# arpg/Kangaroo

Measured on AMD Instinct MI355X. Metric: kinectfusion_frames_per_sec_640x480_to_512cubed_tsdf, higher is better.
Workload: dtype f32

## Files before the change

include/kfx_debug.h:

```cpp
#ifndef KFX_DEBUG_H
#define KFX_DEBUG_H

#include "kfx.h"

#ifdef __cplusplus
extern "C" {
#endif

int kfx_debug_rmw(const kfx_volume* vol, int variant, kfx_stream stream);

int kfx_debug_div_uniform_check(float b, unsigned long long* d_out, kfx_stream stream);

int kfx_debug_div_core_check(unsigned seed, int per_divisor, unsigned long long* d_out, kfx_stream stream);
int kfx_debug_sqrt_core_check(unsigned long long* d_out, kfx_stream stream);
int kfx_debug_wave_xor_check(unsigned seed, unsigned long long* d_out, kfx_stream stream);

int kfx_debug_summary_export(kfx_sdf_summary* s, float tol, float vref, int fine_shift, void* R_out, void* C_out, int dims_out[12],
                             kfx_stream stream);

int kfx_debug_summary_conditional_builds(kfx_sdf_summary* s, int out[2], kfx_stream stream);

#ifdef __cplusplus
}
#endif
#endif
```

kangaroo_amd/csrc/debug.hip:

```cpp
#include "kfx_device.h"
#include "sampling.h"
#include "../../include/kfx_debug.h"

namespace kfx {

__global__ __launch_bounds__(256) void k_rmw_linear(float4* __restrict__ base, size_t n4)
{
    const size_t stride = (size_t)gridDim.x * blockDim.x;
    for (size_t i = (size_t)blockIdx.x * blockDim.x + threadIdx.x; i < n4; i += stride) {
        float4 c = base[i];
        c.y += 1.0f;
        c.w += 1.0f;
        base[i] = c;
    }
}

template <int ZC>
__global__ __launch_bounds__(256) void k_rmw_brick(unsigned char* vptr, size_t pitch, size_t img_pitch, int X, int Y, int Z)
{
    const int tid = threadIdx.x, lane = tid & 63, wv = tid >> 6;
    const int x0 = (blockIdx.x * 32 + (lane & 31)) * 2;
    const int y = blockIdx.y * 8 + wv * 2 + (lane >> 5);
    const int zbeg = blockIdx.z * ZC, zend = min(zbeg + ZC, Z);
    if (x0 >= X || y >= Y) return;
// ... 242 lines not shown
        if (hipMemcpyAsync(C_out, s->C, (size_t)cv.words * sizeof(unsigned), hipMemcpyDeviceToDevice, st) != hipSuccess || hipStreamSynchronize(st) != hipSuccess)
            return set_error(KFX_E_RANGE, "kfx_debug_summary_export: copy");
        dims_out[11] = (s->h_skippable && s->builds) ? ((volatile int*)s->h_skippable)[(s->builds - 1) % KFX_SUMMARY_RING] : -2;
    }
    return 0;
}

extern "C" int kfx_debug_summary_conditional_builds(kfx_sdf_summary* s, int out[2], kfx_stream stream)
{
    if (!s || !out) return set_error(KFX_E_NULL, "kfx_debug_summary_conditional_builds: null argument");
    hipStream_t st = (hipStream_t)stream;
    if (hipMemcpyAsync(out, s->d_count + 3, 2 * sizeof(int), hipMemcpyDeviceToHost, st) != hipSuccess || hipStreamSynchronize(st) != hipSuccess)
        return set_error(KFX_E_RANGE, "kfx_debug_summary_conditional_builds: copy");
    return 0;
}
```

kangaroo_amd/csrc/kfx_device.h:

```cpp
#pragma once

#include <hip/hip_runtime.h>
#include <stddef.h>
#include <stdint.h>

#include "../../include/kfx.h"
#include "../../include/kfx_extras.h"
#include "../../include/kfx_summary_h.h"

namespace kfx {

struct V3 { float x, y, z; };

__device__ __forceinline__ V3 v3(float x, float y, float z) { return V3{x, y, z}; }
__device__ __forceinline__ V3 operator+(V3 a, V3 b) { return V3{a.x + b.x, a.y + b.y, a.z + b.z}; }
__device__ __forceinline__ V3 operator-(V3 a, V3 b) { return V3{a.x - b.x, a.y - b.y, a.z - b.z}; }
__device__ __forceinline__ V3 operator*(V3 a, float s) { return V3{a.x * s, a.y * s, a.z * s}; }
__device__ __forceinline__ V3 div_cw(V3 a, V3 b) { return V3{a.x / b.x, a.y / b.y, a.z / b.z}; }
__device__ __forceinline__ V3 div_s(V3 a, float s) { const float inv = 1.0f / s; return a * inv; }
__device__ __forceinline__ float dot(V3 a, V3 b) { return a.x * b.x + a.y * b.y + a.z * b.z; }
__device__ __forceinline__ float length(V3 a) { return sqrtf(dot(a, a)); }
__device__ __forceinline__ float lerp(float a, float b, float t) { return a + t * (b - a); }
__device__ __forceinline__ V3 lerp(V3 a, V3 b, float t) { return a + (b - a) * t; }
__device__ __forceinline__ float clampf(float f, float a, float b) { return fmaxf(a, fminf(f, b)); }
// ... 141 lines not shown
    int ny;
    int rw;
    int first;
};
struct ClassView {
    const unsigned* C;
    ClassLevel fine, coarse;
    int words;
    float vref;
    float tol;
    int amb_ok;
    int ox, oy, oz;
    float eps;
    int nx5, nz5, top_n, lds_words;
    int global, top_first;
};
__device__ __forceinline__ unsigned brick_class_mask(const float lo, const float hi, const int state, const float lo_ok, const float hi_ok)
{
    const bool in_band = lo >= lo_ok && hi <= hi_ok;
    return (state == 1 ? 1u : 0u) | ((state == 0 && in_band) ? 2u : 0u) | ((state == 1 || in_band) ? 4u : 0u);
}
inline __host__ __device__ void class_level_up(const int nx, const int ny, const int nz, const int shift, const int first, ClassLevel& L, int& ux, int& uz, int& words)
{
    ux = (nx + 1) >> 1; uz = (nz + 1) >> 1;
    L.shift = shift; L.ny = (ny + 1) >> 1; L.rw = 2 * ((ux + 31) >> 5); L.first = first;
    words = (L.rw * L.ny * uz + 3) & ~3;
}
__device__ __forceinline__ void classes_level_up(unsigned* tab, const ClassLevel& src, int snx, int snz, const ClassLevel& dst, int dnx, int dnz)
{
    const int lane = threadIdx.x & 63;
// ... 23 lines not shown
        const unsigned long long p0 = __ballot(cls & 1), p1 = __ballot(cls & 2);
        if (e < total && (bx & 63) == 0 && (chunks > 1 || bx == 0)) {
            const int sh = chunks > 1 ? 0 : lane;
            const unsigned long long m = (chunks > 1 || lg == 6) ? ~0ull : ((1ull << (1 << lg)) - 1ull);
            const unsigned long long r0 = (p0 >> sh) & m, r1 = (p1 >> sh) & m;
            unsigned* out = tab + dst.first + (bz * dst.ny + by) * dst.rw + (bx >> 6) * 4;
            out[0] = (unsigned)r0; out[1] = (unsigned)r1;
            if ((bx >> 6) * 4 + 2 < dst.rw) { out[2] = (unsigned)(r0 >> 32); out[3] = (unsigned)(r1 >> 32); }
        }
    }
}
int summary_classes_prepare(kfx_sdf_summary* s, float tol, float vref, int fine_shift, hipStream_t stream, int global = 0);
void summary_class_layout(const kfx_sdf_summary* s, int fine_shift, ClassView& cv);
void summary_top_layout(const ClassView& cv, ClassLevel& l6, ClassLevel& l7, int& w6, int& w7);
int summary_view_offset(const kfx_sdf_summary* s, const kfx_volume* view, int* ox, int* oy, int* oz);
}

namespace kfx {
int set_error(int code, const char* what);
int check_launch(const char* what);
int math_mode();
size_t texel_image_bytes(size_t w, size_t h);
int depth_to_vbo_normals_texels(const kfx_image* vbo, const kfx_image* nrm, const kfx_image* depth, const float K[4], float scale,
                                const kfx_image* texels, kfx_stream stream);
int sdf_fuse_slab_texels(const kfx_volume* vol, const kfx_slab* slab, const kfx_image* depth, const kfx_image* norm, const kfx_image* texels,
                         const float T_cw[12], const float K[4], float trunc_dist, float max_w, float mincostheta, unsigned flags, kfx_stream stream);
int sdf_fuse_texels(const kfx_volume* vol, kfx_sdf_summary* summary, const kfx_image* depth, const kfx_image* norm, const kfx_image* texels,
                    const float T_cw[12], const float K[4], float trunc_dist, float max_w, float mincostheta, unsigned flags, kfx_stream stream);
}
```

kangaroo_amd/csrc/raycast.hip:

```cpp
#include <cmath>

#include <hip/hip_fp16.h>

#include "kfx_device.h"
#include "sampling.h"

namespace kfx {

struct RayParams {
    VolView vol;
    V3 size;
    V3 dims1;
    V3 hi2;
    V3 voxel;
    V3 inv_size;
    int fastdiv, off32;
    Pose T;
    Intr K;
    unsigned char *dptr, *nptr, *iptr;
    size_t dpitch, npitch, ipitch;
    int w, h;
    float near, far, trunc;
    int subpix;
    int tile_log2w;
    int wg_log2x;
    int sparse_lanes;
};

__device__ __forceinline__ float phong(const V3 p_c, const V3 n_c)
{
    const float ambient = (float)0.4, diffuse = (float)0.4, specular = (float)0.2;
    const V3 eyedir = div_s(p_c * -1.0f, length(p_c));
    const V3 l0 = v3((float)0.4, (float)0.4, -1.0f);
    const V3 lightdir = div_s(l0, length(l0));
    const float ldotn = dot(lightdir, n_c);
    const V3 lightreflect = n_c * (2 * ldotn) + lightdir * -1.0f;
    const float edotr = fmaxf(0.0f, dot(eyedir, lightreflect));
    const float spec = edotr * edotr * edotr * edotr * edotr * edotr * edotr * edotr * edotr * edotr;
    return ambient + diffuse * ldotn + specular * spec;
}

__device__ __forceinline__ void ray_pixel_of(const RayParams& p, int bx, int by, int tid, int& u, int& v)
{
// ... 21 lines not shown
{
    RayBox b;
    b.c_w = v3(p.T.m[3], p.T.m[7], p.T.m[11]);
    b.ray_c = v3(((float)u - p.K.u0) / p.K.fu, ((float)v - p.K.v0) / p.K.fv, 1.0f);
    b.ray_w = so3_mul(p.T, b.ray_c);
    const V3 ta = div_cw(p.vol.bmin - b.c_w, b.ray_w);
    const V3 tb = div_cw(p.vol.bmax - b.c_w, b.ray_w);
    const V3 tmin = v3(fminf(ta.x, tb.x), fminf(ta.y, tb.y), fminf(ta.z, tb.z));
    const V3 tmax = v3(fmaxf(ta.x, tb.x), fmaxf(ta.y, tb.y), fmaxf(ta.z, tb.z));
    b.max_tmin = fmaxf(fmaxf(fmaxf(tmin.x, tmin.y), tmin.z), p.near);
    b.min_tmax = fminf(fminf(fminf(tmax.x, tmax.y), tmax.z), p.far);
    return b;
}
__device__ __forceinline__ bool enters(const RayBox& b) { return b.max_tmin < b.min_tmax; }

template <typename CELL>
__device__ __forceinline__ V3 normal_c(const RayParams& p, const V3 pos_w)
{
    const V3 g = gradient<CELL>(p, pos_w);
    const float len = length(g);
    const V3 n_w = len > 0 ? div_s(g, len) : v3(0.f, 0.f, 1.f);
    return so3_mul_inv(p.T, n_w);
}

struct RayOut { float* depth; float* shade; float4* normal; };
__device__ __forceinline__ RayOut ray_out(const RayParams& p, const int u, const int v)
{
    return RayOut{reinterpret_cast<float*>(p.dptr + (size_t)v * p.dpitch) + u, reinterpret_cast<float*>(p.iptr + (size_t)v * p.ipitch) + u,
                  reinterpret_cast<float4*>(p.nptr + (size_t)v * p.npitch) + u};
}
__device__ __forceinline__ void write_no_hit(const RayOut& o)
{
    *o.depth = __builtin_nanf("");
    *o.shade = 0.f;
    *o.normal = make_float4(0.f, 0.f, 0.f, 0.f);
}
template <typename CELL, bool COLOR>
__device__ __forceinline__ void write_ray(const RayParams& q, const ColorGeom& cv, const int u, const int v, const float depth)
{
    const RayOut o = ray_out(q, u, v);
    if (depth > 0) {
        const RayBox r = ray_box(q, u, v);
        const V3 n_c = normal_c<CELL>(q, r.c_w + r.ray_w * depth);
        *o.depth = depth;
        if constexpr (COLOR) *o.shade = trilinear<RayC32>(cv, r.c_w + r.ray_w * depth);
        else *o.shade = phong(r.ray_c * depth, n_c);
        *o.normal = make_float4(n_c.x, n_c.y, n_c.z, 1.0f);
    } else {
        write_no_hit(o);
    }
}

__device__ __forceinline__ unsigned touch(unsigned* bitmap, const VolView& v, int x, int y, int z)
{
    const size_t i = ((size_t)z * v.h + y) * v.w + x;
    const unsigned bit = 1u << (i & 31);
    unsigned* word = bitmap + (i >> 5);
    if (*reinterpret_cast<volatile unsigned*>(word) & bit) return 0u;
    return (atomicOr(word, bit) & bit) ? 0u : 1u;
}
__device__ __forceinline__ void touch_sample(unsigned* bitmap, const VolView& vol, const CellPos c, unsigned* cnt)
// ... 50 lines not shown
                if (last_sdf > 0) {
                    if (p.subpix) lambda = lambda + delta * sdf / (last_sdf - sdf);
                    depth = lambda;
                }
                break;
            }
            delta = march_step(sdf, min_delta, p.trunc);
            lambda += delta;
            last_sdf = sdf;
        }
    }

    if constexpr (COUNT) {
        if (depth > 0) touch_gradient(bitmap, p, c_w + ray_w * depth, cnt);
    } else {
        write_ray<CELL, COLOR>(p, cv, u, v, depth);
    }
    return depth > 0 ? depth : __builtin_nanf("");
}

struct TopLevels { ClassLevel lv[2]; int n; };

__device__ __forceinline__ int class_lookup(const unsigned* tab, const ClassLevel& L, int gx, int gy, int gz)
{
    const int bx = gx >> L.shift, by = gy >> L.shift, bz = gz >> L.shift;
    const uint2 w = *reinterpret_cast<const uint2*>(tab + L.first + (bz * L.ny + by) * L.rw + ((bx >> 5) << 1));
    return (int)((w.x >> (bx & 31)) & 1u) | (int)(((w.y >> (bx & 31)) & 1u) << 1);
}

template <typename CELL, bool COLOR, bool COUNT = false, bool GT = false>
__device__ __forceinline__ float raycast_pixel_classes(const RayParams& p, const RayParams& q, const ColorGeom& cv, const int u, const int v, const ClassView& cl_arg, const unsigned* tab,
                                                       const TopLevels& top, unsigned* bitmap = nullptr, unsigned* cnt = nullptr)
{
    constexpr bool PARK = !GT && !COUNT;
    ClassView parked;
    if constexpr (PARK) parked = cl_arg;
    ClassView& clp = parked;
    if constexpr (PARK) {
        clp.fine.shift = in_vgpr(clp.fine.shift); clp.fine.ny = in_vgpr(clp.fine.ny); clp.fine.rw = in_vgpr(clp.fine.rw); clp.fine.first = in_vgpr(clp.fine.first);
        clp.coarse.ny = in_vgpr(clp.coarse.ny); clp.coarse.rw = in_vgpr(clp.coarse.rw); clp.coarse.first = in_vgpr(clp.coarse.first);
        clp.ox = in_vgpr(clp.ox); clp.oy = in_vgpr(clp.oy); clp.oz = in_vgpr(clp.oz);
        clp.eps = in_vgpr(clp.eps); clp.vref = in_vgpr(clp.vref);
    }
    const ClassView& cl = PARK ? parked : cl_arg;
    if (u >= p.w || v >= p.h) return 0.f;

    const RayBox box = ray_box(p, u, v);
    const V3 c_w = box.c_w, ray_w = box.ray_w;
    const float max_tmin = box.max_tmin, min_tmax = box.min_tmax;

    float depth = 0.0f;
    if (max_tmin < min_tmax) {
        float lambda = max_tmin;
        float last_sdf = __builtin_nanf("");
        const float min_delta = p.voxel.x;
        float delta = 0.f;
        const V3 sc = v3(p.dims1.x / p.size.x, p.dims1.y / p.size.y, p.dims1.z / p.size.z);
        const V3 pfA = v3((c_w.x - p.vol.bmin.x) * sc.x, (c_w.y - p.vol.bmin.y) * sc.y, (c_w.z - p.vol.bmin.z) * sc.z);
        const V3 pfB = v3(ray_w.x * sc.x, ray_w.y * sc.y, ray_w.z * sc.z);
        const V3 inv = v3(1.0f / pfB.x, 1.0f / pfB.y, 1.0f / pfB.z);
        const float eps = cl.eps;
        const float step_free = fmaxf(cl.vref, min_delta);
        const float inv_step_free = 1.0f / step_free, inv_trunc = 1.0f / p.trunc;
        const float band = cl.tol * cl.vref;
        bool pending = false;
        float lambda_prev = 0.f;
        bool consult = true;
        float lam_retry = lambda;
        int wait = 0, backoff = 1;
        while (lambda < min_tmax) {
            const bool look = consult && wait == 0 && lambda >= lam_retry;
            CellPos c{};
            typename CELL::InFlight fl;
            if (!look) {
                c = cell_of(p, c_w + ray_w * lambda);
                trilinear_issue<CELL>(fl, p, c);
                if constexpr (COUNT) touch_sample(bitmap, p.vol, c, cnt);
            }
            if (look) {
                if constexpr (COUNT) cnt[1] += 1;
                const float ex = __builtin_fmaf(pfB.x, lambda, pfA.x), ey = __builtin_fmaf(pfB.y, lambda, pfA.y), ez = __builtin_fmaf(pfB.z, lambda, pfA.z);
                const float flx = floorf(ex), fly = floorf(ey), flz = floorf(ez);
                const float lo_f = fminf(fminf(ex - flx, ey - fly), ez - flz), hi_f = fmaxf(fmaxf(ex - flx, ey - fly), ez - flz);
                bool run = false;
                if (fminf(fminf(ex, ey), ez) > eps && ex < p.dims1.x - eps && ey < p.dims1.y - eps && ez < p.dims1.z - eps && lo_f > eps && hi_f < 1.0f - eps) {
                    const int gx = (int)flx + cl.ox, gy = (int)fly + cl.oy, gz = (int)flz + cl.oz;
// ... 8 lines not shown
                            int c6 = class_lookup(tab, top.lv[0], gx, gy, gz);
                            if (c6 == 3 && !cl.amb_ok) c6 = 0;
                            if (c6 != 0) { cls = c6; shift = 6; }
                        }
                        if (cls == 0) {
                            int c5 = class_lookup(cl.C, cl.coarse, gx, gy, gz);
                            if (c5 == 3 && !cl.amb_ok) c5 = 0;
                            if (c5 != 0) { cls = c5; shift = 5; }
                        }
                        if (cls == 0) {
                            cls = class_lookup(cl.C, cl.fine, gx, gy, gz);
                            if (cls == 3 && !cl.amb_ok) cls = 0;
                            shift = cl.fine.shift;
                        }
                    } else {
                    cls = class_lookup(tab, cl.fine, gx, gy, gz);
                    if (cls == 3 && !cl.amb_ok) cls = 0;
                    if (cls != 0 && cl.fine.shift < 5) {
                        int c5 = class_lookup(tab, cl.coarse, gx, gy, gz);
                        if (c5 == 3 && !cl.amb_ok) c5 = 0;
                        if (c5 != 0) { cls = c5; shift = 5; }
                    }
                    if (shift == 5 && cl.top_n > 0) {
                        int c6 = class_lookup(tab, top.lv[0], gx, gy, gz);
                        if (c6 == 3 && !cl.amb_ok) c6 = 0;
                        if (c6 != 0) {
                            cls = c6; shift = 6;
                            if (cl.top_n > 1) {
                                int c7 = class_lookup(tab, top.lv[1], gx, gy, gz);
                                if (c7 == 3 && !cl.amb_ok) c7 = 0;
                                if (c7 != 0) { cls = c7; shift = 7; }
                            }
                        }
                    }
                    }
                    const float L = (float)(1 << shift);
                    const float lox = (float)(((gx >> shift) << shift) - cl.ox), loy = (float)(((gy >> shift) << shift) - cl.oy),
                                loz = (float)(((gz >> shift) << shift) - cl.oz);
                    const float bx = pfB.x >= 0.f ? lox + L - eps : lox + eps, by = pfB.y >= 0.f ? loy + L - eps : loy + eps,
                                bz = pfB.z >= 0.f ? loz + L - eps : loz + eps;
                    const float lam_exit = fminf(fminf((bx - pfA.x) * inv.x, (by - pfA.y) * inv.y), (bz - pfA.z) * inv.z);
                    if (cls != 0) {
                        delta = cls == 1 ? step_free : p.trunc;
                        pending = cls == 3 || (CELL::BYTES == 4 && cls == 1 && cl.tol > 0.f);
                        last_sdf = cls == 1 ? cl.vref : __builtin_nanf("");
// ... 28 lines not shown
                        if constexpr (COUNT) touch_sample(bitmap, p.vol, cell_of(p, c_w + ray_w * lambda_prev), cnt);
                    }
                    if (last_sdf > 0) {
                        if (p.subpix) lambda = lambda + delta * sdf / (last_sdf - sdf);
                        depth = lambda;
                    }
                    break;
                }
                delta = march_step(sdf, min_delta, p.trunc);
                lambda += delta;
                last_sdf = sdf;
                pending = false;
                consult = !(fabsf(sdf - cl.vref) > band);
            }
        }
    }

    if constexpr (COUNT) {
        if (depth > 0) touch_gradient(bitmap, p, c_w + ray_w * depth, cnt);
    } else {
        write_ray<CELL, COLOR>(q, cv, u, v, depth);
    }
    return depth > 0 ? depth : __builtin_nanf("");
}

template <bool GT = false>
__device__ __forceinline__ void classes_stage(const ClassView& cl, unsigned* tab, TopLevels& top)
{
    const uint4* src = reinterpret_cast<const uint4*>(cl.C + (GT ? cl.top_first : 0));
    uint4* dst = reinterpret_cast<uint4*>(tab);
    for (int i = threadIdx.x; i < (cl.lds_words >> 2); i += blockDim.x) dst[i] = src[i];
    ClassLevel l6, l7;
    int nx6, nz6, nx7, nz7, w6, w7;
    const int at = GT ? 0 : cl.words;
    class_level_up(cl.nx5, cl.coarse.ny, cl.nz5, 6, at, l6, nx6, nz6, w6);
    class_level_up(nx6, l6.ny, nz6, 7, at + w6, l7, nx7, nz7, w7);
    if (threadIdx.x == 0) { top.lv[0] = l6; top.lv[1] = l7; top.n = cl.top_n; }
    __syncthreads();
}

__device__ __forceinline__ bool workgroup_any(const bool yes, int* s_any)
{
    const bool wave_any = __ballot(yes) != 0ull;
    if ((threadIdx.x & 63) == 0) s_any[threadIdx.x >> 6] = wave_any ? 1 : 0;
    __syncthreads();
    return (s_any[0] | s_any[1] | s_any[2] | s_any[3]) != 0;
}

template <typename CELL, bool GT = false>
__global__ __launch_bounds__(256) void k_raycast_sdf_classes(const RayParams p, const ClassView cl)
{
    extern __shared__ unsigned s_tab[];
    __shared__ RayParams s_p;
    __shared__ TopLevels s_top;
    __shared__ int s_any[4];
    if (threadIdx.x == 0) s_p = p;
    int u, v;
    const bool carries = ray_lane_pixel(p, p.sparse_lanes, blockIdx.x, blockIdx.y, u, v);
    const bool pixel = carries && u < p.w && v < p.h;
    if constexpr (!GT) {
        if (!workgroup_any(pixel && enters(ray_box(p, u, v)), s_any)) {
            if (pixel) write_no_hit(ray_out(p, u, v));
            return;
        }
    }
    classes_stage<GT>(cl, s_tab, s_top);
    if (!carries) return;
    raycast_pixel_classes<CELL, false, false, GT>(p, s_p, ColorGeom{}, u, v, cl, s_tab, s_top);
}

template <typename CELL, bool COLOR>
__global__ __launch_bounds__(256) void k_raycast_sdf(const RayParams p, const ColorGeom cv)
{
    int u, v;
    if (!ray_lane_pixel(p, p.sparse_lanes, blockIdx.x, blockIdx.y, u, v)) return;
    raycast_pixel<CELL, COLOR>(p, cv, u, v);
}

template <typename CELL>
__global__ __launch_bounds__(256) void k_raycast_sdf_count(const RayParams p, unsigned* __restrict__ bitmap, unsigned long long* __restrict__ counters)
{
    int u, v;
    ray_pixel_of(p, blockIdx.x, blockIdx.y, threadIdx.x, u, v);
    unsigned cnt[4] = {0u, 0u, 0u, 0u}, entered = 0;
    if (u < p.w && v < p.h) {
        entered = enters(ray_box(p, u, v)) ? 1u : 0u;
        raycast_pixel<CELL, false, true>(p, ColorGeom{}, u, v, bitmap, cnt);
    }
    publish_counts(cnt, entered, counters);
}

template <typename CELL, bool GT = false>
__global__ __launch_bounds__(256) void k_raycast_sdf_classes_count(const RayParams p, const ClassView cl, unsigned* __restrict__ bitmap,
                                                                   unsigned long long* __restrict__ counters)
{
    extern __shared__ unsigned s_tab[];
    __shared__ RayParams s_p;
    __shared__ TopLevels s_top;
    if (threadIdx.x == 0) s_p = p;
    classes_stage<GT>(cl, s_tab, s_top);
    int u, v;
    ray_pixel_of(p, blockIdx.x, blockIdx.y, threadIdx.x, u, v);
    unsigned cnt[4] = {0u, 0u, 0u, 0u}, entered = 0;
    if (u < p.w && v < p.h) {
        entered = enters(ray_box(p, u, v)) ? 1u : 0u;
        raycast_pixel_classes<CELL, false, true, GT>(p, s_p, ColorGeom{}, u, v, cl, s_tab, s_top, bitmap, cnt);
    }
    publish_counts(cnt, entered, counters);
    if (blockIdx.x == 0 && blockIdx.y == 0 && threadIdx.x == 0) atomicAdd(&counters[5], (unsigned long long)cl.lds_words * 4ull);
}

constexpr int RAY_MAX_LEVELS = 8;
struct RayLevel {
    unsigned char *dptr, *nptr, *iptr;
    size_t dpitch, npitch, ipitch;
    int w, h;
    Intr K;
    unsigned char* vptr;
    size_t vpitch;
    int first_block, blocks_x;
    int sparse;
};
struct RayLevels {
    RayLevel lv[RAY_MAX_LEVELS];
    int n;
};

__device__ __forceinline__ const RayLevel& level_of(const RayLevels& L, const int block)
{
    int l = 0;
    for (int k = 1; k < L.n; ++k)
        if (block >= L.lv[k].first_block) l = k;
    return L.lv[l];
}
__device__ __forceinline__ RayParams level_params(const RayParams& base, const RayLevel& lv)
{
    RayParams p = base;
    p.dptr = lv.dptr; p.nptr = lv.nptr; p.iptr = lv.iptr;
    p.dpitch = lv.dpitch; p.npitch = lv.npitch; p.ipitch = lv.ipitch;
    p.w = lv.w; p.h = lv.h;
    p.K = lv.K;
    return p;
}
__device__ __forceinline__ void write_vertex(const RayLevel& lv, const RayParams& p, const int u, const int v, const float kz)
{
    if (lv.vptr && u < p.w && v < p.h)
        reinterpret_cast<float4*>(lv.vptr + (size_t)v * lv.vpitch)[u] =
            make_float4(kz * ((float)u - p.K.u0) / p.K.fu, kz * ((float)v - p.K.v0) / p.K.fv, kz, 1.0f);
}

template <typename CELL>
__global__ __launch_bounds__(256) void k_raycast_sdf_levels(const RayParams base, const RayLevels L)
{
    const RayLevel& lv = level_of(L, (int)blockIdx.x);
    const RayParams p = level_params(base, lv);
    const int b = (int)blockIdx.x - lv.first_block;
    int u, v;
    if (!ray_lane_pixel(p, lv.sparse, b % lv.blocks_x, b / lv.blocks_x, u, v)) return;
    write_vertex(lv, p, u, v, raycast_pixel<CELL, false>(p, ColorGeom{}, u, v));
}

template <typename CELL>
__global__ __launch_bounds__(256) void k_raycast_sdf_levels_classes(const RayParams base, const RayLevels L, const ClassView cl)
{
    extern __shared__ unsigned s_tab[];
    __shared__ RayParams s_p;
    __shared__ TopLevels s_top;
    __shared__ int s_any[4];
    const RayLevel& lv = level_of(L, (int)blockIdx.x);
    const RayParams p = level_params(base, lv);
    if (threadIdx.x == 0) s_p = p;
    const int b = (int)blockIdx.x - lv.first_block;
    int u, v;
    const bool carries = ray_lane_pixel(p, lv.sparse, b % lv.blocks_x, b / lv.blocks_x, u, v);
    const bool pixel = carries && u < p.w && v < p.h;
    float kz = __builtin_nanf("");
    if (!workgroup_any(pixel && enters(ray_box(p, u, v)), s_any)) {
        if (!pixel) return;
        write_no_hit(ray_out(p, u, v));
    } else {
        classes_stage(cl, s_tab, s_top);
        if (!carries) return;
        kz = raycast_pixel_classes<CELL, false>(p, s_p, ColorGeom{}, u, v, cl, s_tab, s_top);
    }
    write_vertex(lv, p, u, v, kz);
}

struct SlabRay {
    float* state;
    float* touched;
    float* result;
    int packed;
    int normals_here;
    size_t P;
    int R;
    int v0, v1;
    int* fin;
    int claim_misses;
// ... 151 lines not shown
    p.dpitch = depth->pitch;
    p.npitch = norm->pitch;
    p.ipitch = img->pitch;
    p.w = (int)img->w;
    p.h = (int)img->h;
    p.near = near;
    p.far = far;
    p.trunc = trunc_dist;
    p.subpix = subpix ? 1 : 0;
    p.tile_log2w = 5;
    p.wg_log2x = 1;
    p.sparse_lanes = 0;
    return 0;
}

template <typename CELL>
static int class_view(ClassView& cl, size_t* lds_bytes, int* usable, kfx_sdf_summary* summary, const kfx_volume* vol, const RayParams& p, kfx_stream stream,
                      bool allow_global = true)
{
    *usable = 0;
    if (int e = summary_view_offset(summary, vol, &cl.ox, &cl.oy, &cl.oz)) return e;
    if (!(p.trunc > 0.f) || !(p.trunc < __builtin_inff())) return 0;
    static const int kb_env = env_int("KFX_RAYCAST_CLASS_KB", 16, 1, 60);
    static const int gt_env = env_int("KFX_RAYCAST_GLOBAL_TABLES", 0);
    static const int top_env = env_int("KFX_RAYCAST_TOP_LEVELS", 2, 0, 2);
    int fine = 3;
    for (; fine < 5; ++fine) {
        summary_class_layout(summary, fine, cl);
        if ((size_t)cl.words * 4 <= (size_t)kb_env * 1024) break;
    }
// ... 32 lines not shown
    const bool steer = force_env == 0 && summary->h_skippable;
    if (steer && summary->plain_calls && (summary->plain_calls++ % 8u) != 0u) return 0;
    if (int e = summary_classes_prepare(summary, tol, vref, fine, (hipStream_t)stream, cl.global)) return e;
    if (steer && summary->builds >= 3) {
        const unsigned ref = (summary->builds - 3) % KFX_SUMMARY_RING;
        (void)hipEventSynchronize(summary->build_done[ref]);
        const int known = ((volatile int*)summary->h_skippable)[ref];
        if (known >= 0 && (long long)known * 4 < summary->n_coarse) {
            if (!summary->plain_calls) summary->plain_calls = 1;
            return 0;
        }
        summary->plain_calls = 0;
    }
    cl.C = summary->C;
    cl.vref = vref;
    cl.amb_ok = fmaxf(vref, p.voxel.x) == p.trunc ? 1 : 0;
    cl.tol = tol;
    const double u24 = 1.0 / 16777216.0;
    double eps = 0.0;
    const float bmin[3] = {p.vol.bmin.x, p.vol.bmin.y, p.vol.bmin.z}, bmax[3] = {p.vol.bmax.x, p.vol.bmax.y, p.vol.bmax.z};
    const float size[3] = {p.size.x, p.size.y, p.size.z}, dims1[3] = {p.dims1.x, p.dims1.y, p.dims1.z};
    const float cw[3] = {p.T.m[3], p.T.m[7], p.T.m[11]};
    for (int a = 0; a < 3; ++a) {
        if (!(size[a] > 0.f)) return 0;
        const double sc = (double)dims1[a] / size[a];
        const double pmax = std::fmax(std::fabs((double)bmin[a]), std::fabs((double)bmax[a])), ca = std::fabs((double)cw[a]);
        const double A = std::fabs(((double)cw[a] - bmin[a]) * sc);
        const double t = sc * (3.0 * pmax + 2.0 * ca + size[a]) * u24 + 2.0 * dims1[a] * u24;
        const double e = u24 * (3.0 * A + 2.0 * sc * (pmax + ca) + dims1[a]) + 3.0 * u24 * (dims1[a] + A);
        eps = std::fmax(eps, t + e);
// ... 3 lines not shown
    cl.eps = (float)std::fmax(eps, 1e-4);
    *lds_bytes = (size_t)cl.lds_words * sizeof(unsigned);
    *usable = 1;
    return 0;
}

template <typename PLAIN, typename... A>
static int launch_march(const char* what, int usable, const ClassView& cl, size_t cl_bytes, dim3 grid, kfx_stream stream, const RayParams& p,
                        void (*global)(RayParams, ClassView, A...), void (*lds)(RayParams, ClassView, A...), PLAIN plain, A... a)
{
    if (usable) hipLaunchKernelGGL(cl.global ? global : lds, grid, dim3(256), cl_bytes, (hipStream_t)stream, p, cl, a...);
    else plain();
    return check_launch(what);
}

template <typename CELL>
static int raycast_levels_launch(int n_levels, const kfx_image* const* depth, const kfx_image* const* norm, const kfx_image* const* img,
                                 const kfx_image* const* vbo, const kfx_volume* vol, const float T_wc[12], const float* K, float near, float far,
                                 float trunc_dist, int subpix, kfx_stream stream, kfx_sdf_summary* summary = nullptr)
{
    if (n_levels < 0 || n_levels > RAY_MAX_LEVELS) return set_error(KFX_E_RANGE, "RaycastSdf(levels): number of levels");
    if (!depth || !norm || !img || !K) return set_error(KFX_E_NULL, "RaycastSdf(levels): null argument");
    RayParams base{};
    RayLevels L{};
    int blocks = 0;
    for (int l = 0; l < n_levels; ++l) {
        RayParams p;
        if (int e = ray_params<CELL>(p, depth[l], norm[l], img[l], vol, T_wc, K + 4 * l, near, far, trunc_dist, subpix)) return e;
        if (p.w == 0 || p.h == 0) continue;
        RayLevel& lv = L.lv[L.n++];
// ... 298 lines not shown
}

extern "C" int kfx_raycast_state_to_images(const kfx_image* depth, const kfx_image* norm, const kfx_image* img, const float* state,
                                           kfx_stream stream)
{
    if (!depth || !norm || !img || !state || !depth->ptr || !norm->ptr || !img->ptr) return set_error(KFX_E_NULL, "raycast state: null argument");
    if (img->w == 0 || img->h == 0) return 0;
    if (depth->w < img->w || depth->h < img->h || norm->w < img->w || norm->h < img->h) return set_error(KFX_E_SHAPE, "raycast state: image sizes");
    RayParams p{};
    p.dptr = (unsigned char*)depth->ptr; p.nptr = (unsigned char*)norm->ptr; p.iptr = (unsigned char*)img->ptr;
    p.dpitch = depth->pitch; p.npitch = norm->pitch; p.ipitch = img->pitch;
    p.w = (int)img->w; p.h = (int)img->h;
    hipLaunchKernelGGL(k_raycast_state_to_images, dim3(ceil_div(p.w, 64), ceil_div(p.h, 4)), dim3(256), 0, (hipStream_t)stream, p, state);
    return check_launch("kfx_raycast_state_to_images");
}
```

kangaroo_amd/csrc/sampling.h:

```cpp
#pragma once

#include <hip/hip_fp16.h>

#include "kfx_device.h"
#include "host_args.h"

namespace kfx {

struct __attribute__((aligned(8))) Pair { float v0, w0, v1, w1; };
struct RayF32 {
    static constexpr int BYTES = 8;
    __device__ static __forceinline__ float2 pair(const unsigned char* row, int x)
    {
        const Pair c = *reinterpret_cast<const Pair*>(row + (size_t)x * 8);
        return make_float2(c.v0, c.v1);
    }
    __device__ static __forceinline__ float val(const unsigned char* row, int x) { return *reinterpret_cast<const float*>(row + (size_t)x * 8); }
    __device__ static __forceinline__ void pair4(const unsigned char* base, size_t o0, size_t o1, size_t o2, size_t o3,
                                                 float2& c0, float2& c1, float2& c2, float2& c3)
    {
        typedef float f4 __attribute__((ext_vector_type(4)));
        f4 a, b, c, d;
        asm volatile("global_load_dwordx4 %0, %4, off\n\t"
                     "global_load_dwordx4 %1, %5, off\n\t"
// ... 195 lines not shown
__device__ __forceinline__ float trilinear_finish(typename CELL::InFlight& f, const CellPos& c)
{
    float2 c00, c10, c01, c11;
    CELL::finish(f, c00, c10, c01, c11);
    return lerp(lerp(lerp(c00.x, c00.y, c.fx), lerp(c10.x, c10.y, c.fx), c.fy),
                lerp(lerp(c01.x, c01.y, c.fx), lerp(c11.x, c11.y, c.fx), c.fy), c.fz);
}

template <typename CELL, typename GEOM>
__device__ __forceinline__ float trilinear(const GEOM& p, const V3 pos_w)
{
    return trilinear_at<CELL>(p, cell_of(p, pos_w));
}

template <typename CELL, typename GEOM>
__device__ __forceinline__ V3 gradient(const GEOM& p, const V3 pos_w)
{
    const V3 pos_v = div_cw(pos_w - p.vol.bmin, p.size);
    const V3 pf = v3(pos_v.x * p.dims1.x, pos_v.y * p.dims1.y, pos_v.z * p.dims1.z);
    const int ix = (int)fmaxf(fminf(p.hi2.x, floorf(pf.x)), 1.f);
    const int iy = (int)fmaxf(fminf(p.hi2.y, floorf(pf.y)), 1.f);
    const int iz = (int)fmaxf(fminf(p.hi2.z, floorf(pf.z)), 1.f);
    const float fx = pf.x - (float)ix, fy = pf.y - (float)iy, fz = pf.z - (float)iz;
    const VolView& v = p.vol;
    float c[2][2][2], mx[2][2], my[2][2], mz[2][2];
#pragma unroll
    for (int dz = 0; dz < 2; ++dz)
#pragma unroll
        for (int dy = 0; dy < 2; ++dy) {
            const unsigned char* r = rowp(v, iy + dy, iz + dz);
            mx[dz][dy] = CELL::val(r, ix - 1);
            const float2 cc = CELL::pair(r, ix);
            c[dz][dy][0] = cc.x;
// ... 14 lines not shown
    V3 g[2][2][2];
#pragma unroll
    for (int dz = 0; dz < 2; ++dz)
#pragma unroll
        for (int dy = 0; dy < 2; ++dy)
#pragma unroll
            for (int dx = 0; dx < 2; ++dx) {
                const float v0 = c[dz][dy][dx];
                const float bx = dx ? c[dz][dy][0] : mx[dz][dy];
                const float by = dy ? c[dz][0][dx] : my[dz][dx];
                const float bz = dz ? c[0][dy][dx] : mz[dy][dx];
                g[dz][dy][dx] = v3(v0 - bx, v0 - by, v0 - bz);
            }
    const V3 deriv = lerp(lerp(lerp(g[0][0][0], g[0][0][1], fx), lerp(g[0][1][0], g[0][1][1], fx), fy),
                          lerp(lerp(g[1][0][0], g[1][0][1], fx), lerp(g[1][1][0], g[1][1][1], fx), fy), fz);
    return div_cw(deriv, p.voxel);
}

template <typename GEOM>
inline void set_shortcuts(GEOM& g)
{
    g.inv_size = V3{1.0f / g.size.x, 1.0f / g.size.y, 1.0f / g.size.z};
    g.fastdiv = div_uniform_safe_host(g.size.x) && div_uniform_safe_host(g.size.y) && div_uniform_safe_host(g.size.z);
    const double span = (double)(g.vol.d - 1) * (double)g.vol.img_pitch + (double)(g.vol.h - 1) * (double)g.vol.pitch + (double)g.vol.w * 16.0;
    static const int enabled = env_int("KFX_SAMPLER_SHORTCUTS", 1);
    g.off32 = enabled && span < 4294967296.0;
    g.fastdiv = enabled && g.fastdiv;
}

template <typename GEOM>
inline void set_geometry(GEOM& g, const kfx_volume* v)
// ... 22 lines not shown
```

Baseline: 2476.

## Prefetch class table early, hoist march quotients, spread params copy across threads

In the class-table raycast kernels, the first chunk of the class table is loaded into registers before the ray-box test and workgroup vote, so global latency overlaps that work before the LDS store. RayParams is now copied to LDS one word per thread instead of by thread 0 alone. Per-ray constants (scale, free step, reciprocals) are computed on the host and passed in ClassView, the ray box is computed once and passed down, and class words for all pyramid levels are loaded together before they are tested. A clock-instrumented debug variant is added behind a compile flag; the prefetch uses more registers and loads table words even for blocks that then exit early.

```diff
diff --git a/include/kfx_debug.h b/include/kfx_debug.h
--- a/include/kfx_debug.h
+++ b/include/kfx_debug.h
@@ -20,6 +20,12 @@
 
 int kfx_debug_summary_conditional_builds(kfx_sdf_summary* s, int out[2], kfx_stream stream);
 
+int kfx_debug_march_clocks(const kfx_image* depth, const kfx_image* norm, const kfx_image* img, const kfx_volume* vol, kfx_sdf_summary* summary,
+                           const float T_wc[12], const float K[4], float near, float far, float trunc_dist, int subpix,
+                           unsigned long long* d_clocks, size_t clock_words, int* waves, kfx_stream stream);
+
+int kfx_debug_march_quotients(const float boxmin[3], const float boxmax[3], const unsigned dims[3], float trunc_dist, float vref, float out[6]);
+
 #ifdef __cplusplus
 }
 #endif
diff --git a/kangaroo_amd/csrc/debug.hip b/kangaroo_amd/csrc/debug.hip
--- a/kangaroo_amd/csrc/debug.hip
+++ b/kangaroo_amd/csrc/debug.hip
@@ -280,3 +280,11 @@
         return set_error(KFX_E_RANGE, "kfx_debug_summary_conditional_builds: copy");
     return 0;
 }
+
+extern "C" int kfx_debug_march_quotients(const float boxmin[3], const float boxmax[3], const unsigned dims[3], float trunc_dist, float vref, float out[6])
+{
+    if (!boxmin || !boxmax || !dims || !out) return set_error(KFX_E_NULL, "kfx_debug_march_quotients: null argument");
+    if (dims[0] < 3 || dims[1] < 3 || dims[2] < 3) return set_error(KFX_E_SHAPE, "kfx_debug_march_quotients: a volume has at least 3 cells per axis");
+    march_quotients_of(boxmin, boxmax, dims, trunc_dist, vref, out);
+    return 0;
+}
diff --git a/kangaroo_amd/csrc/kfx_device.h b/kangaroo_amd/csrc/kfx_device.h
--- a/kangaroo_amd/csrc/kfx_device.h
+++ b/kangaroo_amd/csrc/kfx_device.h
@@ -179,6 +179,8 @@
     float eps;
     int nx5, nz5, top_n, lds_words;
     int global, top_first;
+    V3 sc;
+    float step_free, inv_step_free, inv_trunc;
 };
 __device__ __forceinline__ unsigned brick_class_mask(const float lo, const float hi, const int state, const float lo_ok, const float hi_ok)
 {
@@ -232,6 +234,7 @@
 void summary_class_layout(const kfx_sdf_summary* s, int fine_shift, ClassView& cv);
 void summary_top_layout(const ClassView& cv, ClassLevel& l6, ClassLevel& l7, int& w6, int& w7);
 int summary_view_offset(const kfx_sdf_summary* s, const kfx_volume* view, int* ox, int* oy, int* oz);
+void march_quotients_of(const float bmin[3], const float bmax[3], const unsigned dims[3], float trunc_dist, float vref, float out[6]);
 }
 
 namespace kfx {
diff --git a/kangaroo_amd/csrc/raycast.hip b/kangaroo_amd/csrc/raycast.hip
--- a/kangaroo_amd/csrc/raycast.hip
+++ b/kangaroo_amd/csrc/raycast.hip
@@ -27,6 +27,14 @@
     int sparse_lanes;
 };
 
+#ifdef KFX_MARCH_CLOCKS
+constexpr int MARCH_CLOCK_WORDS = 8;
+__device__ __forceinline__ void clock_stamp(unsigned long long* rec, const int slot) { rec[slot] = wall_clock64(); }
+#define KFX_CLOCK_STAMP(rec, slot) clock_stamp(rec, slot)
+#else
+#define KFX_CLOCK_STAMP(rec, slot) ((void)0)
+#endif
+
 __device__ __forceinline__ float phong(const V3 p_c, const V3 n_c)
 {
     const float ambient = (float)0.4, diffuse = (float)0.4, specular = (float)0.2;
@@ -78,10 +86,10 @@
 }
 __device__ __forceinline__ bool enters(const RayBox& b) { return b.max_tmin < b.min_tmax; }
 
-template <typename CELL>
+template <typename CELL, bool UNIFORM_DIV = false>
 __device__ __forceinline__ V3 normal_c(const RayParams& p, const V3 pos_w)
 {
-    const V3 g = gradient<CELL>(p, pos_w);
+    const V3 g = UNIFORM_DIV ? gradient_uniform<CELL>(p, pos_w) : gradient<CELL>(p, pos_w);
     const float len = length(g);
     const V3 n_w = len > 0 ? div_s(g, len) : v3(0.f, 0.f, 1.f);
     return so3_mul_inv(p.T, n_w);
@@ -99,16 +107,16 @@
     *o.shade = 0.f;
     *o.normal = make_float4(0.f, 0.f, 0.f, 0.f);
 }
-template <typename CELL, bool COLOR>
-__device__ __forceinline__ void write_ray(const RayParams& q, const ColorGeom& cv, const int u, const int v, const float depth)
+template <typename CELL, bool COLOR, bool UNIFORM_DIV = false>
+__device__ __forceinline__ void write_ray(const RayParams& q, const ColorGeom& cv, const int u, const int v, const V3 ray_c, const V3 ray_w, const float depth)
 {
     const RayOut o = ray_out(q, u, v);
     if (depth > 0) {
-        const RayBox r = ray_box(q, u, v);
-        const V3 n_c = normal_c<CELL>(q, r.c_w + r.ray_w * depth);
+        const V3 c_w = v3(q.T.m[3], q.T.m[7], q.T.m[11]);
+        const V3 n_c = normal_c<CELL, UNIFORM_DIV>(q, c_w + ray_w * depth);
         *o.depth = depth;
-        if constexpr (COLOR) *o.shade = trilinear<RayC32>(cv, r.c_w + r.ray_w * depth);
-        else *o.shade = phong(r.ray_c * depth, n_c);
+        if constexpr (COLOR) *o.shade = trilinear<RayC32>(cv, c_w + ray_w * depth);
+        else *o.shade = phong(ray_c * depth, n_c);
         *o.normal = make_float4(n_c.x, n_c.y, n_c.z, 1.0f);
     } else {
         write_no_hit(o);
@@ -189,7 +197,7 @@
     if constexpr (COUNT) {
         if (depth > 0) touch_gradient(bitmap, p, c_w + ray_w * depth, cnt);
     } else {
-        write_ray<CELL, COLOR>(p, cv, u, v, depth);
+        write_ray<CELL, COLOR>(p, cv, u, v, box.ray_c, ray_w, depth);
     }
     return depth > 0 ? depth : __builtin_nanf("");
 }
@@ -202,10 +210,26 @@
     const uint2 w = *reinterpret_cast<const uint2*>(tab + L.first + (bz * L.ny + by) * L.rw + ((bx >> 5) << 1));
     return (int)((w.x >> (bx & 31)) & 1u) | (int)(((w.y >> (bx & 31)) & 1u) << 1);
 }
+__device__ __forceinline__ uint2 class_words(const unsigned* tab, const ClassLevel& L, int gx, int gy, int gz)
+{
+    const int bx = gx >> L.shift, by = gy >> L.shift, bz = gz >> L.shift;
+    return *reinterpret_cast<const uint2*>(tab + L.first + (bz * L.ny + by) * L.rw + ((bx >> 5) << 1));
+}
+__device__ __forceinline__ int class_in(const uint2 w, const int shift, const int gx, const int amb_ok)
+{
+    const int bx = gx >> shift;
+    const int c = (int)((w.x >> (bx & 31)) & 1u) | (int)(((w.y >> (bx & 31)) & 1u) << 1);
+    return (c == 3 && !amb_ok) ? 0 : c;
+}
 
 template <typename CELL, bool COLOR, bool COUNT = false, bool GT = false>
-__device__ __forceinline__ float raycast_pixel_classes(const RayParams& p, const RayParams& q, const ColorGeom& cv, const int u, const int v, const ClassView& cl_arg, const unsigned* tab,
-                                                       const TopLevels& top, unsigned* bitmap = nullptr, unsigned* cnt = nullptr)
+__device__ __forceinline__ float raycast_pixel_classes(const RayParams& p, const RayParams& q, const ColorGeom& cv, const int u, const int v, const RayBox& box,
+                                                       const ClassView& cl_arg, const unsigned* tab, const TopLevels& top, unsigned* bitmap = nullptr,
+                                                       unsigned* cnt = nullptr
+#ifdef KFX_MARCH_CLOCKS
+                                                       , unsigned long long* wave_rec = nullptr
+#endif
+                                                       )
 {
     constexpr bool PARK = !GT && !COUNT;
     ClassView parked;
@@ -218,10 +242,13 @@
         clp.eps = in_vgpr(clp.eps); clp.vref = in_vgpr(clp.vref);
     }
     const ClassView& cl = PARK ? parked : cl_arg;
+    const V3 sc = v3(in_vgpr(cl_arg.sc.x), in_vgpr(cl_arg.sc.y), in_vgpr(cl_arg.sc.z));
+    const float step_free = in_vgpr(cl_arg.step_free);
+    const float inv_step_free = in_vgpr(cl_arg.inv_step_free), inv_trunc = in_vgpr(cl_arg.inv_trunc);
     if (u >= p.w || v >= p.h) return 0.f;
 
-    const RayBox box = ray_box(p, u, v);
     const V3 c_w = box.c_w, ray_w = box.ray_w;
+    const float ray_cx = box.ray_c.x, ray_cy = box.ray_c.y;
     const float max_tmin = box.max_tmin, min_tmax = box.min_tmax;
 
     float depth = 0.0f;
@@ -230,21 +257,24 @@
         float last_sdf = __builtin_nanf("");
         const float min_delta = p.voxel.x;
         float delta = 0.f;
-        const V3 sc = v3(p.dims1.x / p.size.x, p.dims1.y / p.size.y, p.dims1.z / p.size.z);
         const V3 pfA = v3((c_w.x - p.vol.bmin.x) * sc.x, (c_w.y - p.vol.bmin.y) * sc.y, (c_w.z - p.vol.bmin.z) * sc.z);
         const V3 pfB = v3(ray_w.x * sc.x, ray_w.y * sc.y, ray_w.z * sc.z);
         const V3 inv = v3(1.0f / pfB.x, 1.0f / pfB.y, 1.0f / pfB.z);
         const float eps = cl.eps;
-        const float step_free = fmaxf(cl.vref, min_delta);
-        const float inv_step_free = 1.0f / step_free, inv_trunc = 1.0f / p.trunc;
         const float band = cl.tol * cl.vref;
         bool pending = false;
         float lambda_prev = 0.f;
         bool consult = true;
         float lam_retry = lambda;
         int wait = 0, backoff = 1;
+#ifdef KFX_MARCH_CLOCKS
+        unsigned n_look = 0, n_sample = 0;
+#endif
         while (lambda < min_tmax) {
             const bool look = consult && wait == 0 && lambda >= lam_retry;
+#ifdef KFX_MARCH_CLOCKS
+            n_look += look ? 1u : 0u; n_sample += look ? 0u : 1u;
+#endif
             CellPos c{};
             typename CELL::InFlight fl;
             if (!look) {
@@ -283,21 +313,23 @@
                             shift = cl.fine.shift;
                         }
                     } else {
-                    cls = class_lookup(tab, cl.fine, gx, gy, gz);
-                    if (cls == 3 && !cl.amb_ok) cls = 0;
-                    if (cls != 0 && cl.fine.shift < 5) {
-                        int c5 = class_lookup(tab, cl.coarse, gx, gy, gz);
-                        if (c5 == 3 && !cl.amb_ok) c5 = 0;
+                    const bool has5 = cl_arg.fine.shift < 5, has6 = cl_arg.top_n > 0, has7 = cl_arg.top_n > 1;
+                    const uint2 wf = class_words(tab, cl.fine, gx, gy, gz);
+                    uint2 w5 = wf, w6 = wf, w7 = wf;
+                    if (has5) w5 = class_words(tab, cl.coarse, gx, gy, gz);
+                    if (has6) w6 = class_words(tab, top.lv[0], gx, gy, gz);
+                    if (has7) w7 = class_words(tab, top.lv[1], gx, gy, gz);
+                    cls = class_in(wf, cl.fine.shift, gx, cl.amb_ok);
+                    if (has5 && cls != 0) {
+                        const int c5 = class_in(w5, 5, gx, cl.amb_ok);
                         if (c5 != 0) { cls = c5; shift = 5; }
                     }
-                    if (shift == 5 && cl.top_n > 0) {
-                        int c6 = class_lookup(tab, top.lv[0], gx, gy, gz);
-                        if (c6 == 3 && !cl.amb_ok) c6 = 0;
+                    if (has6 && shift == 5) {
+                        const int c6 = class_in(w6, 6, gx, cl.amb_ok);
                         if (c6 != 0) {
                             cls = c6; shift = 6;
-                            if (cl.top_n > 1) {
-                                int c7 = class_lookup(tab, top.lv[1], gx, gy, gz);
-                                if (c7 == 3 && !cl.amb_ok) c7 = 0;
+                            if (has7) {
+                                const int c7 = class_in(w7, 7, gx, cl.amb_ok);
                                 if (c7 != 0) { cls = c7; shift = 7; }
                             }
                         }
@@ -356,22 +388,49 @@
                 consult = !(fabsf(sdf - cl.vref) > band);
             }
         }
-    }
+#ifdef KFX_MARCH_CLOCKS
+        if (wave_rec) {
+            atomicMax(&wave_rec[5], (unsigned long long)n_look); atomicMax(&wave_rec[6], (unsigned long long)n_sample);
+            atomicMax(&wave_rec[7], (unsigned long long)(n_look + n_sample));
+        }
+#endif
+    }
+#ifdef KFX_MARCH_CLOCKS
+    if (wave_rec) clock_stamp(wave_rec, 3);
+#endif
 
     if constexpr (COUNT) {
         if (depth > 0) touch_gradient(bitmap, p, c_w + ray_w * depth, cnt);
     } else {
-        write_ray<CELL, COLOR>(q, cv, u, v, depth);
+        write_ray<CELL, COLOR, true>(q, cv, u, v, v3(ray_cx, ray_cy, 1.0f), ray_w, depth);
     }
     return depth > 0 ? depth : __builtin_nanf("");
 }
 
+constexpr int STAGE_EARLY = 4;
+struct StagedWords { uint4 w[STAGE_EARLY]; };
+__device__ __forceinline__ void classes_request(const ClassView& cl, StagedWords& e)
+{
+    const uint4* src = reinterpret_cast<const uint4*>(cl.C);
+    const int n = cl.lds_words >> 2;
+#pragma unroll
+    for (int k = 0; k < STAGE_EARLY; ++k) {
+        const int i = (int)threadIdx.x + k * 256;
+        e.w[k] = i < n ? src[i] : make_uint4(0u, 0u, 0u, 0u);
+    }
+}
 template <bool GT = false>
-__device__ __forceinline__ void classes_stage(const ClassView& cl, unsigned* tab, TopLevels& top)
+__device__ __forceinline__ void classes_stage(const ClassView& cl, unsigned* tab, TopLevels& top, const StagedWords* early = nullptr)
 {
     const uint4* src = reinterpret_cast<const uint4*>(cl.C + (GT ? cl.top_first : 0));
     uint4* dst = reinterpret_cast<uint4*>(tab);
-    for (int i = threadIdx.x; i < (cl.lds_words >> 2); i += blockDim.x) dst[i] = src[i];
+    int i = threadIdx.x;
+    if (early) {
+#pragma unroll
+        for (int k = 0; k < STAGE_EARLY; ++k, i += 256)
+            if (i < (cl.lds_words >> 2)) dst[i] = early->w[k];
+    }
+    for (; i < (cl.lds_words >> 2); i += blockDim.x) dst[i] = src[i];
     ClassLevel l6, l7;
     int nx6, nz6, nx7, nz7, w6, w7;
     const int at = GT ? 0 : cl.words;
@@ -381,6 +440,17 @@
     __syncthreads();
 }
 
+static_assert(sizeof(RayParams) % 4 == 0 && sizeof(RayParams) / 4 <= 256, "one word per thread of the workgroup");
+__device__ __forceinline__ unsigned params_word(const RayParams& src)
+{
+    return threadIdx.x < sizeof(RayParams) / 4 ? reinterpret_cast<const unsigned*>(&src)[threadIdx.x] : 0u;
+}
+__device__ __forceinline__ void params_word_to_lds(RayParams& dst, const unsigned word)
+{
+    if (threadIdx.x < sizeof(RayParams) / 4) reinterpret_cast<unsigned*>(&dst)[threadIdx.x] = word;
+}
+__device__ __forceinline__ void params_to_lds(RayParams& dst, const RayParams& src) { params_word_to_lds(dst, params_word(src)); }
+
 __device__ __forceinline__ bool workgroup_any(const bool yes, int* s_any)
 {
     const bool wave_any = __ballot(yes) != 0ull;
@@ -390,25 +460,50 @@
 }
 
 template <typename CELL, bool GT = false>
+#ifdef KFX_MARCH_CLOCKS
+__global__ __launch_bounds__(256) void k_raycast_sdf_classes(const RayParams p, const ClassView cl, unsigned long long* clocks)
+#else
 __global__ __launch_bounds__(256) void k_raycast_sdf_classes(const RayParams p, const ClassView cl)
-{
+#endif
+{
+#ifdef KFX_MARCH_CLOCKS
+    unsigned long long* const rec = clocks + ((size_t)(blockIdx.y * gridDim.x + blockIdx.x) * 4 + (threadIdx.x >> 6)) * MARCH_CLOCK_WORDS;
+#endif
+    KFX_CLOCK_STAMP(rec, 0);
     extern __shared__ unsigned s_tab[];
     __shared__ RayParams s_p;
     __shared__ TopLevels s_top;
     __shared__ int s_any[4];
-    if (threadIdx.x == 0) s_p = p;
+    const unsigned p_word = params_word(p);
     int u, v;
     const bool carries = ray_lane_pixel(p, p.sparse_lanes, blockIdx.x, blockIdx.y, u, v);
     const bool pixel = carries && u < p.w && v < p.h;
+    RayBox box;
     if constexpr (!GT) {
-        if (!workgroup_any(pixel && enters(ray_box(p, u, v)), s_any)) {
+        StagedWords early;
+        classes_request(cl, early);
+        box = ray_box(p, u, v);
+        params_word_to_lds(s_p, p_word);
+        if (!workgroup_any(pixel && enters(box), s_any)) {
             if (pixel) write_no_hit(ray_out(p, u, v));
+            KFX_CLOCK_STAMP(rec, 1); KFX_CLOCK_STAMP(rec, 4);
             return;
         }
-    }
-    classes_stage<GT>(cl, s_tab, s_top);
+        KFX_CLOCK_STAMP(rec, 1);
+        classes_stage<GT>(cl, s_tab, s_top, &early);
+        KFX_CLOCK_STAMP(rec, 2);
+    } else {
+        params_word_to_lds(s_p, p_word);
+        classes_stage<GT>(cl, s_tab, s_top);
+        box = ray_box(p, u, v);
+    }
     if (!carries) return;
-    raycast_pixel_classes<CELL, false, false, GT>(p, s_p, ColorGeom{}, u, v, cl, s_tab, s_top);
+#ifdef KFX_MARCH_CLOCKS
+    raycast_pixel_classes<CELL, false, false, GT>(p, s_p, ColorGeom{}, u, v, box, cl, s_tab, s_top, nullptr, nullptr, rec);
+    clock_stamp(rec, 4);
+#else
+    raycast_pixel_classes<CELL, false, false, GT>(p, s_p, ColorGeom{}, u, v, box, cl, s_tab, s_top);
+#endif
 }
 
 template <typename CELL, bool COLOR>
@@ -439,14 +534,15 @@
     extern __shared__ unsigned s_tab[];
     __shared__ RayParams s_p;
     __shared__ TopLevels s_top;
-    if (threadIdx.x == 0) s_p = p;
+    params_to_lds(s_p, p);
     classes_stage<GT>(cl, s_tab, s_top);
     int u, v;
     ray_pixel_of(p, blockIdx.x, blockIdx.y, threadIdx.x, u, v);
     unsigned cnt[4] = {0u, 0u, 0u, 0u}, entered = 0;
     if (u < p.w && v < p.h) {
-        entered = enters(ray_box(p, u, v)) ? 1u : 0u;
-        raycast_pixel_classes<CELL, false, true, GT>(p, s_p, ColorGeom{}, u, v, cl, s_tab, s_top, bitmap, cnt);
+        const RayBox box = ray_box(p, u, v);
+        entered = enters(box) ? 1u : 0u;
+        raycast_pixel_classes<CELL, false, true, GT>(p, s_p, ColorGeom{}, u, v, box, cl, s_tab, s_top, bitmap, cnt);
     }
     publish_counts(cnt, entered, counters);
     if (blockIdx.x == 0 && blockIdx.y == 0 && threadIdx.x == 0) atomicAdd(&counters[5], (unsigned long long)cl.lds_words * 4ull);
@@ -475,13 +571,17 @@
         if (block >= L.lv[k].first_block) l = k;
     return L.lv[l];
 }
-__device__ __forceinline__ RayParams level_params(const RayParams& base, const RayLevel& lv)
-{
-    RayParams p = base;
+__device__ __forceinline__ void level_override(RayParams& p, const RayLevel& lv)
+{
     p.dptr = lv.dptr; p.nptr = lv.nptr; p.iptr = lv.iptr;
     p.dpitch = lv.dpitch; p.npitch = lv.npitch; p.ipitch = lv.ipitch;
     p.w = lv.w; p.h = lv.h;
     p.K = lv.K;
+}
+__device__ __forceinline__ RayParams level_params(const RayParams& base, const RayLevel& lv)
+{
+    RayParams p = base;
+    level_override(p, lv);
     return p;
 }
 __device__ __forceinline__ void write_vertex(const RayLevel& lv, const RayParams& p, const int u, const int v, const float kz)
@@ -511,19 +611,24 @@
     __shared__ int s_any[4];
     const RayLevel& lv = level_of(L, (int)blockIdx.x);
     const RayParams p = level_params(base, lv);
-    if (threadIdx.x == 0) s_p = p;
+    const unsigned p_word = params_word(base);
     const int b = (int)blockIdx.x - lv.first_block;
     int u, v;
     const bool carries = ray_lane_pixel(p, lv.sparse, b % lv.blocks_x, b / lv.blocks_x, u, v);
     const bool pixel = carries && u < p.w && v < p.h;
     float kz = __builtin_nanf("");
-    if (!workgroup_any(pixel && enters(ray_box(p, u, v)), s_any)) {
+    StagedWords early;
+    classes_request(cl, early);
+    const RayBox box = ray_box(p, u, v);
+    params_word_to_lds(s_p, p_word);
+    if (threadIdx.x == 0) level_override(s_p, lv);
+    if (!workgroup_any(pixel && enters(box), s_any)) {
         if (!pixel) return;
         write_no_hit(ray_out(p, u, v));
     } else {
-        classes_stage(cl, s_tab, s_top);
+        classes_stage(cl, s_tab, s_top, &early);
         if (!carries) return;
-        kz = raycast_pixel_classes<CELL, false>(p, s_p, ColorGeom{}, u, v, cl, s_tab, s_top);
+        kz = raycast_pixel_classes<CELL, false>(p, s_p, ColorGeom{}, u, v, box, cl, s_tab, s_top);
     }
     write_vertex(lv, p, u, v, kz);
 }
@@ -705,6 +810,31 @@
     return 0;
 }
 
+static void march_quotients(ClassView& cl, const RayParams& p, const float vref)
+{
+    cl.sc = V3{p.dims1.x / p.size.x, p.dims1.y / p.size.y, p.dims1.z / p.size.z};
+    cl.step_free = fmaxf(vref, p.voxel.x);
+    cl.inv_step_free = 1.0f / cl.step_free;
+    cl.inv_trunc = 1.0f / p.trunc;
+}
+#ifndef KFX_MARCH_CLOCKS
+namespace kfx {
+void march_quotients_of(const float bmin[3], const float bmax[3], const unsigned dims[3], const float trunc_dist, const float vref, float out[6])
+{
+    kfx_volume v{};
+    v.w = dims[0]; v.h = dims[1]; v.d = dims[2];
+    for (int a = 0; a < 3; ++a) { v.boxmin[a] = bmin[a]; v.boxmax[a] = bmax[a]; }
+    RayParams p{};
+    set_geometry(p, &v);
+    set_voxel_size(p, &v);
+    p.trunc = trunc_dist;
+    ClassView cl{};
+    march_quotients(cl, p, vref);
+    out[0] = cl.sc.x; out[1] = cl.sc.y; out[2] = cl.sc.z; out[3] = cl.step_free; out[4] = cl.inv_step_free; out[5] = cl.inv_trunc;
+}
+}
+#endif
+
 template <typename CELL>
 static int class_view(ClassView& cl, size_t* lds_bytes, int* usable, kfx_sdf_summary* summary, const kfx_volume* vol, const RayParams& p, kfx_stream stream,
                       bool allow_global = true)
@@ -767,6 +897,7 @@
     }
     cl.C = summary->C;
     cl.vref = vref;
+    march_quotients(cl, p, vref);
     cl.amb_ok = fmaxf(vref, p.voxel.x) == p.trunc ? 1 : 0;
     cl.tol = tol;
     const double u24 = 1.0 / 16777216.0;
@@ -800,6 +931,33 @@
     return check_launch(what);
 }
 
+#ifdef KFX_MARCH_CLOCKS
+extern "C" int kfx_debug_march_clocks(const kfx_image* depth, const kfx_image* norm, const kfx_image* img, const kfx_volume* vol, kfx_sdf_summary* summary,
+                                      const float T_wc[12], const float K[4], float near, float far, float trunc_dist, int subpix,
+                                      unsigned long long* d_clocks, size_t clock_words, int* waves, kfx_stream stream)
+{
+    if (!summary || !waves) return set_error(KFX_E_NULL, "kfx_debug_march_clocks: null argument");
+    RayParams p;
+    if (int e = ray_params<RayF32>(p, depth, norm, img, vol, T_wc, K, near, far, trunc_dist, subpix)) return e;
+    if (summary->cell_bytes != RayF32::BYTES || p.w == 0 || p.h == 0) return set_error(KFX_E_SHAPE, "kfx_debug_march_clocks: an fp32 summary and a non-empty image");
+    const dim3 grid(ceil_div(p.w, 64), ceil_div(p.h, 4));
+    *waves = (int)(grid.x * grid.y * 4);
+    if (!d_clocks) return 0;
+    if (clock_words < (size_t)*waves * MARCH_CLOCK_WORDS) return set_error(KFX_E_SHAPE, "kfx_debug_march_clocks: 8 words per wave");
+    ClassView cl;
+    size_t cl_bytes = 0;
+    int usable = 0;
+    const unsigned plain_calls = summary->plain_calls;
+    const int ce = class_view<RayF32>(cl, &cl_bytes, &usable, summary, vol, p, stream);
+    summary->plain_calls = plain_calls;
+    if (ce) return ce;
+    if (!usable || cl.global) return set_error(KFX_E_RANGE, "kfx_debug_march_clocks: this call would not run the LDS-mode table march");
+    if (hipMemsetAsync(d_clocks, 0, (size_t)*waves * MARCH_CLOCK_WORDS * sizeof(unsigned long long), (hipStream_t)stream) != hipSuccess)
+        return set_error(KFX_E_RANGE, "kfx_debug_march_clocks: memset");
+    hipLaunchKernelGGL((k_raycast_sdf_classes<RayF32, false>), grid, dim3(256), cl_bytes, (hipStream_t)stream, p, cl, d_clocks);
+    return check_launch("kfx_debug_march_clocks");
+}
+#else
 template <typename CELL>
 static int raycast_levels_launch(int n_levels, const kfx_image* const* depth, const kfx_image* const* norm, const kfx_image* const* img,
                                  const kfx_image* const* vbo, const kfx_volume* vol, const float T_wc[12], const float* K, float near, float far,
@@ -1128,3 +1286,4 @@
     hipLaunchKernelGGL(k_raycast_state_to_images, dim3(ceil_div(p.w, 64), ceil_div(p.h, 4)), dim3(256), 0, (hipStream_t)stream, p, state);
     return check_launch("kfx_raycast_state_to_images");
 }
+#endif
diff --git a/kangaroo_amd/csrc/sampling.h b/kangaroo_amd/csrc/sampling.h
--- a/kangaroo_amd/csrc/sampling.h
+++ b/kangaroo_amd/csrc/sampling.h
@@ -233,9 +233,8 @@
 }
 
 template <typename CELL, typename GEOM>
-__device__ __forceinline__ V3 gradient(const GEOM& p, const V3 pos_w)
-{
-    const V3 pos_v = div_cw(pos_w - p.vol.bmin, p.size);
+__device__ __forceinline__ V3 gradient_cells(const GEOM& p, const V3 pos_v)
+{
     const V3 pf = v3(pos_v.x * p.dims1.x, pos_v.y * p.dims1.y, pos_v.z * p.dims1.z);
     const int ix = (int)fmaxf(fminf(p.hi2.x, floorf(pf.x)), 1.f);
     const int iy = (int)fmaxf(fminf(p.hi2.y, floorf(pf.y)), 1.f);
@@ -280,7 +279,17 @@
             }
     const V3 deriv = lerp(lerp(lerp(g[0][0][0], g[0][0][1], fx), lerp(g[0][1][0], g[0][1][1], fx), fy),
                           lerp(lerp(g[1][0][0], g[1][0][1], fx), lerp(g[1][1][0], g[1][1][1], fx), fy), fz);
-    return div_cw(deriv, p.voxel);
+    return deriv;
+}
+template <typename CELL, typename GEOM>
+__device__ __forceinline__ V3 gradient(const GEOM& p, const V3 pos_w)
+{
+    return div_cw(gradient_cells<CELL>(p, div_cw(pos_w - p.vol.bmin, p.size)), p.voxel);
+}
+template <typename CELL, typename GEOM>
+__device__ __forceinline__ V3 gradient_uniform(const GEOM& p, const V3 pos_w)
+{
+    return div_cw(gradient_cells<CELL>(p, box_fraction(p, pos_w)), p.voxel);
 }
 
 template <typename GEOM>
```

Result: no change. 2488 (median of 6 runs) (+0.5%).
